# Andreas-Edling/raytracer-rs

Hardware: AMD Instinct MI355X
Metric: Mrays/s (whole node) + ms/frame, 1920x1080x64spp thai2.dae (higher is better)
Workload: dtype f32

## Files before the change

### raytracer-rs_amd/csrc/lightmap.cpp

```cpp
#include "lightmap.hpp"
#include <algorithm>
#include <cmath>
#include <cstring>
#include <limits>

namespace mi355rt {
namespace {

struct V3 { double x, y, z; };
inline V3 sub(V3 a, V3 b) { return { a.x - b.x, a.y - b.y, a.z - b.z }; }
inline V3 add(V3 a, V3 b) { return { a.x + b.x, a.y + b.y, a.z + b.z }; }
inline V3 mul(V3 a, double s) { return { a.x * s, a.y * s, a.z * s }; }
inline double dot(V3 a, V3 b) { return a.x * b.x + a.y * b.y + a.z * b.z; }
inline V3 cross(V3 a, V3 b) { return { a.y * b.z - a.z * b.y, a.z * b.x - a.x * b.z, a.x * b.y - a.y * b.x }; }
inline double len(V3 a) { return std::sqrt(dot(a, a)); }
inline double comp(V3 a, int k) { return k == 0 ? a.x : k == 1 ? a.y : a.z; }

double origin_triangle_distance(V3 a, V3 b, V3 c)
{
    const V3 ab = sub(b, a), ac = sub(c, a), ap = mul(a, -1.0);
    const double d1 = dot(ab, ap), d2 = dot(ac, ap);
    if (d1 <= 0.0 && d2 <= 0.0) return len(a);
    const V3 bp = mul(b, -1.0);
    const double d3 = dot(ab, bp), d4 = dot(ac, bp);
    if (d3 >= 0.0 && d4 <= d3) return len(b);
    const double vc = d1 * d4 - d3 * d2;
    if (vc <= 0.0 && d1 >= 0.0 && d3 <= 0.0) return len(add(a, mul(ab, d1 / (d1 - d3))));
    const V3 cp = mul(c, -1.0);
    const double d5 = dot(ab, cp), d6 = dot(ac, cp);
    if (d6 >= 0.0 && d5 <= d6) return len(c);
    const double vb = d5 * d2 - d1 * d6;
    if (vb <= 0.0 && d2 >= 0.0 && d6 <= 0.0) return len(add(a, mul(ac, d2 / (d2 - d6))));
    const double va = d3 * d6 - d5 * d4;
    if (va <= 0.0 && (d4 - d3) >= 0.0 && (d5 - d6) >= 0.0) return len(add(b, mul(sub(c, b), (d4 - d3) / ((d4 - d3) + (d5 - d6)))));
    const double den = va + vb + vc;
    if (!(std::fabs(den) > 0.0)) return -1.0;
    const double v = vb / den, w = vc / den;
    return len(add(a, add(mul(ab, v), mul(ac, w))));
}

template <class F> int clip(const V3* in, int n, V3* out, F f)
{
    int m = 0;
    for (int i = 0; i < n; ++i) {
        const V3 A = in[i], B = in[(i + 1) % n];
        const double fa = f(A), fb = f(B);
        if (fa >= 0.0) out[m++] = A;
        if ((fa >= 0.0) != (fb >= 0.0)) { const double t = fa / (fa - fb); out[m++] = add(A, mul(sub(B, A), t)); }
    }
    return m;
}

inline float round_down(double v)
{
    float f = (float)v;
    if ((double)f > v) f = std::nextafterf(f, 0.0f);
    return f;
}

}

static const int kAxisA[3] = { 1, 0, 0 }, kAxisB[3] = { 2, 2, 1 };

void build_light_map(const float* tri_verts, uint32_t ntri, const float light[3], double pad, uint32_t res, LightMap& out)
{
    const uint32_t R = res;
    out.res = R;
    out.dist2.assign((size_t)6 * R * R, std::numeric_limits<float>::infinity());
    out.nearest = std::numeric_limits<double>::infinity();
    const V3 L = { light[0], light[1], light[2] };
    const double rho = std::sqrt(2.0) / (double)R * 1.001;
    const double cos_rho = std::cos(rho), sin_rho = std::sin(rho);
    for (uint32_t t = 0; t < ntri; ++t) {
        const float* v = tri_verts + 9 * (size_t)t;
        const V3 P[3] = { sub({ v[0], v[1], v[2] }, L), sub({ v[3], v[4], v[5] }, L), sub({ v[6], v[7], v[8] }, L) };
        double dmin = origin_triangle_distance(P[0], P[1], P[2]);
        {
            const double size = std::max(len(sub(P[1], P[0])), std::max(len(sub(P[2], P[0])), len(sub(P[2], P[1]))));
            const double near_vertex = std::min(len(P[0]), std::min(len(P[1]), len(P[2])));
            const double lower = std::max(near_vertex - size, 0.0);
            if (!(dmin >= 0.0) || !std::isfinite(dmin)) dmin = lower;
            dmin = std::min(std::max(dmin, lower), near_vertex);
            if (!(dmin == dmin)) dmin = 0.0;
        }
        out.nearest = std::min(out.nearest, dmin);
        const V3 n = cross(sub(P[1], P[0]), sub(P[2], P[0]));
        const double nn = len(n);
        const bool has_plane = nn > 0.0 && std::isfinite(nn);
        double h = 0.0; V3 nh = { 0, 0, 0 };
        if (has_plane) { const double c = dot(n, P[0]) / nn; h = std::fabs(c); nh = mul(n, (c < 0.0 ? -1.0 : 1.0) / nn); }
        for (int face = 0; face < 6; ++face) {
            const int m = face >> 1, a = kAxisA[m], b = kAxisB[m];
            const double sg = (face & 1) ? -1.0 : 1.0;
            V3 poly[2][16]; int np = 3;
            poly[0][0] = P[0]; poly[0][1] = P[1]; poly[0][2] = P[2];
            const double eps = 1e-12 * (1.0 + len(P[0])), dl = 1e-6;
            int cur = 0;
            np = clip(poly[cur], np, poly[cur ^ 1], [&](V3 q) { return sg * comp(q, m) - eps; }); cur ^= 1; if (np == 0) continue;
            np = clip(poly[cur], np, poly[cur ^ 1], [&](V3 q) { return sg * comp(q, m) * (1.0 + dl) - comp(q, a); }); cur ^= 1; if (np == 0) continue;
            np = clip(poly[cur], np, poly[cur ^ 1], [&](V3 q) { return sg * comp(q, m) * (1.0 + dl) + comp(q, a); }); cur ^= 1; if (np == 0) continue;
            np = clip(poly[cur], np, poly[cur ^ 1], [&](V3 q) { return sg * comp(q, m) * (1.0 + dl) - comp(q, b); }); cur ^= 1; if (np == 0) continue;
            np = clip(poly[cur], np, poly[cur ^ 1], [&](V3 q) { return sg * comp(q, m) * (1.0 + dl) + comp(q, b); }); cur ^= 1; if (np == 0) continue;
            double u0 = 1e300, u1 = -1e300, v0 = 1e300, v1 = -1e300, mmin = 1e300;
            for (int k = 0; k < np; ++k) {
                const double mm = sg * comp(poly[cur][k], m);
                if (!(mm > 0.0)) { mmin = 0.0; continue; }
                mmin = std::min(mmin, mm);
                const double uu = comp(poly[cur][k], a) / mm, vv = comp(poly[cur][k], b) / mm;
                u0 = std::min(u0, uu); u1 = std::max(u1, uu); v0 = std::min(v0, vv); v1 = std::max(v1, vv);
            }
            long i0 = 0, i1 = (long)R - 1, j0 = 0, j1 = (long)R - 1;
            if (mmin > 0.0 && u0 <= u1) {
                const double mu = 2.5 * pad / mmin + 1e-7;
                i0 = (long)std::floor((std::max(u0 - mu, -1.0) * 0.5 + 0.5) * R - 0.01); i1 = (long)std::floor((std::min(u1 + mu, 1.0) * 0.5 + 0.5) * R + 0.01);
                j0 = (long)std::floor((std::max(v0 - mu, -1.0) * 0.5 + 0.5) * R - 0.01); j1 = (long)std::floor((std::min(v1 + mu, 1.0) * 0.5 + 0.5) * R + 0.01);
                i0 = std::max(i0, 0L); j0 = std::max(j0, 0L); i1 = std::min(i1, (long)R - 1); j1 = std::min(j1, (long)R - 1);
            }
            float* fm = out.dist2.data() + (size_t)face * R * R;
            for (long i = i0; i <= i1; ++i) {
                const double uc = ((double)i + 0.5) / R * 2.0 - 1.0;
                for (long j = j0; j <= j1; ++j) {
                    double lb = dmin;
                    if (has_plane) {
                        const double vc = ((double)j + 0.5) / R * 2.0 - 1.0;
                        double w[3]; w[m] = sg; w[a] = uc; w[b] = vc;
                        const double wl = std::sqrt(w[0] * w[0] + w[1] * w[1] + w[2] * w[2]);
                        const double cos_c = (w[0] * nh.x + w[1] * nh.y + w[2] * nh.z) / wl;
                        if (cos_c > -0.999999) {
                            const double sin_c = std::sqrt(std::max(0.0, 1.0 - cos_c * cos_c));
                            const double cos_lo = cos_c >= cos_rho ? 1.0 : cos_c * cos_rho + sin_c * sin_rho;
                            if (cos_lo > 1e-4) lb = std::max(lb, h / cos_lo);
                            else lb = std::max(lb, h * 1e4);
                        }
                    }
                    const double d = std::max(lb - pad, 0.0);
                    const float val = round_down(d * d * (1.0 - 1e-6));
                    float& dst = fm[(size_t)i * R + (size_t)j];
                    if (val < dst) dst = val;
                }
            }
        }
    }
}

double point_triangle_distance_lower(const double p[3], const float* v)
{
    const V3 L = { p[0], p[1], p[2] };
    const V3 P[3] = { sub({ v[0], v[1], v[2] }, L), sub({ v[3], v[4], v[5] }, L), sub({ v[6], v[7], v[8] }, L) };
    double dmin = origin_triangle_distance(P[0], P[1], P[2]);
    const double size = std::max(len(sub(P[1], P[0])), std::max(len(sub(P[2], P[0])), len(sub(P[2], P[1]))));
    const double near_vertex = std::min(len(P[0]), std::min(len(P[1]), len(P[2])));
    const double lower = std::max(near_vertex - size, 0.0);
    if (!(dmin >= 0.0) || !std::isfinite(dmin)) dmin = lower;
    dmin = std::min(std::max(dmin, lower), near_vertex);
    return dmin == dmin ? dmin : 0.0;
}

uint64_t light_map_work(const float* tri_verts, uint32_t ntri, const float light[3], uint32_t res)
{
    const V3 L = { light[0], light[1], light[2] };
    double total = 0.0;
    for (uint32_t t = 0; t < ntri; ++t) {
        const float* v = tri_verts + 9 * (size_t)t;
        const V3 P[3] = { sub({ v[0], v[1], v[2] }, L), sub({ v[3], v[4], v[5] }, L), sub({ v[6], v[7], v[8] }, L) };
        const V3 c = mul(add(P[0], add(P[1], P[2])), 1.0 / 3.0);
        const double r = std::max(len(sub(P[0], c)), std::max(len(sub(P[1], c)), len(sub(P[2], c)))), d = len(c);
        double frac = 1.0;
        if (d > r * 1.0001) { const double s = r / d; frac = std::min(1.0, s * s * 0.5 + 4.0 / ((double)res * res)); }
        total += frac * 6.0 * (double)res * res;
    }
    return (uint64_t)std::min(total, 1e18);
}

}
```

### raytracer-rs_amd/csrc/reflmask.hpp

```cpp
#pragma once
#include <cstdint>
#include <vector>

namespace mi355rt {

constexpr double kReflMinCos = 0.05;
constexpr double kReflPadAngle = 1e-3;
constexpr float kReflBary = 0.02f;
constexpr double kReflHeightUlps = 16.0;
constexpr uint32_t kReflBins = 8;
constexpr uint32_t kReflGuardWords = 4;

struct ReflMask {
    uint32_t bins = 0;
    uint32_t stride = 0;
    std::vector<uint32_t> words;
    double build_ms = 0.0;
    uint64_t work = 0;
    uint64_t exact_tests = 0;
    uint64_t clear_bits = 0;
};

inline uint32_t refl_mask_stride(uint32_t bins) { return 6u * bins * bins / 32u + kReflGuardWords; }

bool build_reflect_mask(const float* tri_verts, uint32_t ntri, double pad, uint32_t bins, uint64_t work_budget, ReflMask& out,
                        double min_cos = kReflMinCos, double pad_angle = kReflPadAngle);

}
```

### raytracer-rs_amd/csrc/renderer.cpp

```cpp
#include "renderer.hpp"
#include "display.hpp"
#include "lightmap.hpp"
#include "reflmask.hpp"
#include <algorithm>
#include <array>
#include <chrono>
#include <cmath>
#include <cstdio>
#include <cstdlib>
#include <cstring>
#include "kernels.hpp"
#include "lens.hpp"
#include "octree.hpp"

namespace mi355rt {

namespace {
void pcg4d(uint32_t v[4])
{
    for (int i = 0; i < 4; ++i) v[i] = v[i] * 1664525u + 1013904223u;
    v[0] += v[1] * v[3]; v[1] += v[2] * v[0]; v[2] += v[0] * v[1]; v[3] += v[1] * v[2];
    for (int i = 0; i < 4; ++i) v[i] ^= v[i] >> 16;
    v[0] += v[1] * v[3]; v[1] += v[2] * v[0]; v[2] += v[0] * v[1]; v[3] += v[1] * v[2];
}
float u01(uint32_t bits) { return (float)(bits >> 9) * (1.0f / 8388608.0f); }
}

bool Renderer::fail(hipError_t e, const char* what)
{
    last_error = std::string(what) + ": " + hipGetErrorString(e);
    return false;
}
#define HIP_TRY(expr) do { hipError_t e__ = (expr); if (e__ != hipSuccess) return fail(e__, #expr); } while (0)

bool Renderer::bind()
{
    HIP_TRY(hipSetDevice(cfg.device));
    return true;
}

template <class T> bool Renderer::upload(DeviceBuffer<T>& buf, const void* src, size_t bytes)
{
    HIP_TRY(buf.alloc(bytes ? bytes : 16, &hbm_bytes_));
    if (bytes && src) HIP_TRY(hipMemcpy(buf.get(), src, bytes, hipMemcpyHostToDevice));
    else if (bytes) HIP_TRY(hipMemset(buf.get(), 0, bytes));
    return true;
}

template <class T> bool Renderer::upload(T*& dptr, const void* src, size_t bytes)
{
    scene_bufs_.emplace_back();
    if (!upload(scene_bufs_.back(), src, bytes)) return false;
    dptr = static_cast<T*>(scene_bufs_.back().get());
    return true;
}

std::unique_ptr<Renderer> Renderer::create(const SceneData& scene, const mi355rt_config& cfg, std::string& err, int& code)
{
    std::unique_ptr<Renderer> r(new Renderer());
    r->cfg = cfg;
    if (!r->init(scene, err, code)) return nullptr;
    return r;
}

void Renderer::build_sample_table(std::vector<float>& table4)
{
    table.resize((size_t)kNumSamples * 3);
    table4.assign((size_t)kNumSamples * 4, 0.0f);
    for (uint32_t i = 0; i < kNumSamples; ++i) {
        for (uint32_t attempt = 0;; ++attempt) {
            uint32_t h[4] = { i, attempt, 0xFFFFFFFFu, (uint32_t)cfg.seed };
            pcg4d(h);
            Vec3 d(u01(h[0]) * 2.0f + -1.0f, u01(h[1]) * 2.0f + -1.0f, u01(h[2]) * 2.0f + -1.0f);
            if (dot(d, d) < 1.0f) {
                Vec3 nrm = d.normalized();
                table[3 * (size_t)i] = nrm.x; table[3 * (size_t)i + 1] = nrm.y; table[3 * (size_t)i + 2] = nrm.z;
                table4[4 * (size_t)i] = nrm.x; table4[4 * (size_t)i + 1] = nrm.y; table4[4 * (size_t)i + 2] = nrm.z;
                break;
            }
        }
    }
}

bool Renderer::set_seed(uint64_t seed)
{
    if (!bind()) return false;
    if (!settle_speculation()) return false;
    cfg.seed = seed;
    std::vector<float> table4;
    build_sample_table(table4);
    for (Slice& o : slices_) if (o.stream) HIP_TRY(hipStreamSynchronize(o.stream));
    HIP_TRY(hipMemcpy(const_cast<void*>(dscene_.table), table4.data(), table4.size() * sizeof(float), hipMemcpyHostToDevice));
    return true;
}

bool Renderer::set_flags(uint32_t flags)
{
    constexpr uint32_t kCreateMask = MI355RT_FLAG_OCTREE_SEMANTICS | MI355RT_FLAG_TRUE_CLOSEST_HIT | MI355RT_FLAG_GROUP_SHARES_DEVICE | MI355RT_FLAG_DEVICE_LBVH | MI355RT_FLAG_DIRECT_FILM;
    if ((flags ^ cfg.flags) & kCreateMask) { last_error = "the intersector flags (OCTREE_SEMANTICS, TRUE_CLOSEST_HIT), GROUP_SHARES_DEVICE, DEVICE_LBVH and DIRECT_FILM are create-time flags: they cannot be changed with mi355rt_set_flags"; return false; }
    if (flags != cfg.flags && !settle_speculation()) return false;
    cfg.flags = flags;
    return true;
}

bool Renderer::init(const SceneData& scene, std::string& err, int& code)
{
    code = MI355RT_E_INVALID;
    if (cfg.recursions == 0 && cfg.spread == 0) { cfg.recursions = 2; cfg.spread = 1; }
    if (cfg.spread == 0) cfg.spread = 1;
    if (cfg.triangles_per_leaf == 0) cfg.triangles_per_leaf = MI355RT_DEFAULT_TRIANGLES_PER_LEAF;
    if (cfg.width == 0 || cfg.height == 0) { err = "width and height must be non-zero"; return false; }
    if ((uint64_t)cfg.width * cfg.height > 0x7FFFFFFFull / 4) { err = "image too large"; return false; }
    if (cfg.recursions > kMaxRecursions) { err = "recursions > 3 not supported"; return false; }
    if (scene.cameras.empty()) { err = "scene has no camera"; return false; }
    if (scene.tri_geom.size() * 9 != scene.tri_verts.size()) { err = "tri_verts / tri_geom size mismatch"; return false; }
    for (uint32_t g : scene.tri_geom) if (g >= scene.materials.size()) { err = "tri_geom entry out of range"; return false; }
    for (auto& m : scene.materials) if (m.kind == 1 && m.tex_id >= scene.textures.size()) { err = "material texture id out of range"; return false; }
    if (scene.tri_geom.size() >= (1u << 26)) { err = "too many triangles"; return false; }
    {
        uint64_t count = 1, first = 0;
        for (uint32_t l = 0; l <= cfg.recursions; ++l) {
            level_first[l] = (uint32_t)first; first += count; count *= (uint64_t)cfg.spread * (cfg.recursions - l);
            if (first > 0xFFFF) { err = "radiance tree too large (spread * recursions)"; return false; }
        }
        for (uint32_t l = cfg.recursions + 1; l <= kMaxLevels; ++l) level_first[l] = (uint32_t)first;
        nodes_per_sample = (uint32_t)first;
    }
    if (cfg.stripe_world <= 1) { cfg.stripe_world = 1; cfg.stripe_rank = 0; }
    if (cfg.stripe_rows == 0) cfg.stripe_rows = MI355RT_DEFAULT_STRIPE_ROWS;
    if (cfg.stripe_rank >= cfg.stripe_world) { err = "stripe_rank >= stripe_world"; return false; }

    code = MI355RT_E_NO_DEVICE;
    int ndev = 0;
    hipError_t e = hipGetDeviceCount(&ndev);
    if (e != hipSuccess || ndev <= 0) { err = std::string("no HIP device available (") + hipGetErrorString(e) + "); this library has no CPU fallback"; return false; }
    if (cfg.device < 0 || cfg.device >= ndev) { err = "HIP device ordinal out of range"; return false; }
    auto bail = [&]() { err = last_error; return false; };
    if (!bind()) return bail();
    hipDeviceProp_t prop;
    if (hipGetDeviceProperties(&prop, cfg.device) != hipSuccess) { err = "hipGetDeviceProperties failed"; return false; }
    num_cus_ = prop.multiProcessorCount > 0 ? prop.multiProcessorCount : 256;
    if (hipStreamCreateWithFlags(&stream_, hipStreamNonBlocking) != hipSuccess) { err = "hipStreamCreate failed"; return false; }
    if (hipEventCreate(&ev_begin_) != hipSuccess || hipEventCreate(&ev_end_) != hipSuccess) { err = "hipEventCreate failed"; return false; }

    ntri = scene.ntri();
    nlights_ = (uint32_t)scene.lights.size();
    camera = Camera::from_orientation_matrix(cfg.width, cfg.height, Matrix::from_array(scene.cameras[0].orientation), scene.cameras[0].fov_deg);

    const auto t_bvh = std::chrono::steady_clock::now();
    bool on_device = false;
    if (cfg.flags & MI355RT_FLAG_DEVICE_LBVH) {
        std::string why; double ms[2];
        on_device = build_bvh_device(scene.tri_verts.data(), scene.tri_geom.data(), ntri, bvh, why, ms);
        if (on_device) { lbvh_device_ms_ = ms[0]; }
        else last_error = "device LBVH not used (" + why + "): host SAH build instead";
    }
    if (!on_device) build_bvh(scene.tri_verts.data(), scene.tri_geom.data(), ntri, bvh);
    bvh_on_device_ = on_device;
    wide_ = false;
    if (kernels_walk_wide_nodes()) {
        build_wide(bvh);
        if (!bvh.nodes4.empty()) wide_ = true;
        else if (bvh.root >= 0) { err = "this build's kernels walk the 4-wide tree, which does not serve this scene"; code = MI355RT_E_INVALID; return false; }
    }
    build_ms_[0] = std::chrono::duration<double, std::milli>(std::chrono::steady_clock::now() - t_bvh).count();
    collect_cull_boxes();
    if (bvh.max_depth > kBvhMaxDepth) { err = "internal: BVH deeper than the traversal stack"; code = MI355RT_E_INVALID; return false; }
    std::vector<float> normals((size_t)std::max(ntri, 1u) * 4, 0.0f);
    for (uint32_t t = 0; t < ntri; ++t) {
        const float* v = &scene.tri_verts[9 * (size_t)t];
        Vec3 v0(v[0], v[1], v[2]), v1(v[3], v[4], v[5]), v2(v[6], v[7], v[8]);
        Vec3 n = cross(v1 - v0, v2 - v0).normalized();
        normals[4 * (size_t)t] = n.x; normals[4 * (size_t)t + 1] = n.y; normals[4 * (size_t)t + 2] = n.z;
        uint32_t g = scene.tri_geom[t];
        std::memcpy(&normals[4 * (size_t)t + 3], &g, 4);
    }
    std::vector<float> table4;
    build_sample_table(table4);
    void* d_nodes = nullptr; void* d_tris = nullptr; void* d_normals = nullptr; void* d_table = nullptr;
    DMaterial* d_mats = nullptr; DLight* d_lights = nullptr; DTexture* d_tex = nullptr; float* d_texels = nullptr;
    if (wide_ ? !upload(d_nodes, bvh.nodes4.data(), bvh.nodes4.size() * sizeof(BvhNode4)) : !upload(d_nodes, bvh.nodes.data(), bvh.nodes.size() * sizeof(BvhNode))) return bail();
    if (!upload(d_tris, bvh.tris.data(), bvh.tris.size() * sizeof(BvhTri))) return bail();
    if (!upload(d_normals, normals.data(), normals.size() * sizeof(float))) return bail();
    if (!upload(d_table, table4.data(), table4.size() * sizeof(float))) return bail();
    std::vector<DMaterial> mats(std::max<size_t>(scene.materials.size(), 1));
    for (size_t i = 0; i < scene.materials.size(); ++i) {
        const MaterialData& m = scene.materials[i];
        mats[i] = DMaterial{ m.rgb[0], m.rgb[1], m.rgb[2], m.kind == 1 ? (0x80000000u | m.tex_id) : 0u };
    }
    if (!upload(d_mats, mats.data(), mats.size() * sizeof(DMaterial))) return bail();
    std::vector<DLight> lights(std::max<size_t>(scene.lights.size(), 1));
    for (size_t i = 0; i < scene.lights.size(); ++i) {
        const LightData& l = scene.lights[i];
        lights[i] = DLight{ l.pos[0], l.pos[1], l.pos[2], l.color[0], l.color[1], l.color[2], 0.0f, 0.0f };
    }
    float* d_light_maps = nullptr; uint32_t light_map_res = 0;
    if (!scene.lights.empty() && scene.lights.size() <= 8 && ntri > 0 && !getenv("MI355RT_NO_LIGHT_MAP")) {
        const auto t_lm = std::chrono::steady_clock::now();
        double diag2 = 0.0;
        { float mn[3] = { 3e38f, 3e38f, 3e38f }, mx[3] = { -3e38f, -3e38f, -3e38f };
          for (size_t i = 0; i < scene.tri_verts.size(); ++i) { const int a = (int)(i % 3); mn[a] = std::min(mn[a], scene.tri_verts[i]); mx[a] = std::max(mx[a], scene.tri_verts[i]); }
          for (int a = 0; a < 3; ++a) diag2 += ((double)mx[a] - mn[a]) * ((double)mx[a] - mn[a]); }
        const double pad = 2e-4 * std::sqrt(diag2) + 1e-7;
        uint32_t res = 512;
        while (res > 16 && (size_t)6 * res * res * 4 * scene.lights.size() > ((size_t)64 << 20)) res /= 2;
        const uint64_t work_cap = 4ull << 20;
        for (const LightData& l : scene.lights) while (res > 16 && light_map_work(scene.tri_verts.data(), ntri, l.pos, res) > work_cap) res /= 2;
        std::vector<float> all; all.reserve((size_t)6 * res * res * scene.lights.size());
        bool finite = true;
        for (size_t i = 0; i < scene.lights.size() && finite; ++i) {
            const LightData& l = scene.lights[i];
            if (!std::isfinite(l.pos[0]) || !std::isfinite(l.pos[1]) || !std::isfinite(l.pos[2])) { finite = false; break; }
            LightMap lm; build_light_map(scene.tri_verts.data(), ntri, l.pos, pad, res, lm);
            all.insert(all.end(), lm.dist2.begin(), lm.dist2.end());
            const double tail = std::max(lm.nearest - pad, 0.0);
            lights[i].tail2 = std::isfinite(tail) ? (float)std::min(tail * tail * (1.0 - 1e-6), 3.0e38) : 3.0e38f;
            if ((double)lights[i].tail2 > tail * tail) lights[i].tail2 = std::nextafterf(lights[i].tail2, 0.0f);
        }
        if (finite) {
            if (!upload(d_light_maps, all.data(), all.size() * sizeof(float))) return bail();
            light_map_res = res;
        }
        light_map_ms_ = std::chrono::duration<double, std::milli>(std::chrono::steady_clock::now() - t_lm).count();
        if (getenv("MI355RT_DEBUG_CULL")) fprintf(stderr, "[mi355rt] light maps: %zu lights, %u texels per face edge, %.1f ms\n", scene.lights.size(), light_map_res, light_map_ms_);
    }
    if (!upload(d_lights, lights.data(), lights.size() * sizeof(DLight))) return bail();
    uint32_t* d_refl_mask = nullptr; uint32_t refl_bins = 0, refl_stride = 0;
    if (ntri > 0 && cfg.recursions > 0 && !getenv("MI355RT_NO_REFLECT_MASK")) {
        double diag2 = 0.0;
        { float mn[3] = { 3e38f, 3e38f, 3e38f }, mx[3] = { -3e38f, -3e38f, -3e38f };
          for (size_t i = 0; i < scene.tri_verts.size(); ++i) { const int a = (int)(i % 3); mn[a] = std::min(mn[a], scene.tri_verts[i]); mx[a] = std::max(mx[a], scene.tri_verts[i]); }
          for (int a = 0; a < 3; ++a) diag2 += ((double)mx[a] - mn[a]) * ((double)mx[a] - mn[a]); }
        uint64_t budget = 4000000000ull;
        if (const char* e = getenv("MI355RT_REFLECT_MASK_WORK")) budget = std::strtoull(e, nullptr, 10);
        ReflMask rm;
        if (std::isfinite(diag2) && build_reflect_mask(scene.tri_verts.data(), ntri, 2e-4 * std::sqrt(diag2) + 1e-7, kReflBins, budget, rm)) {
            if (!upload(d_refl_mask, rm.words.data(), rm.words.size() * sizeof(uint32_t))) return bail();
            refl_bins = rm.bins; refl_stride = rm.stride;
            reflect_mask_info_[2] = (double)rm.clear_bits / ((double)ntri * 6.0 * rm.bins * rm.bins);
            reflect_mask_info_[3] = (double)(rm.words.size() * sizeof(uint32_t));
        }
        reflect_mask_info_[0] = (double)refl_bins; reflect_mask_info_[1] = rm.build_ms;
        if (getenv("MI355RT_DEBUG_CULL")) fprintf(stderr, "[mi355rt] reflection masks: %u bins per face edge, %.1f ms, %llu work units, %.3f of the bits clear\n", refl_bins, rm.build_ms, (unsigned long long)rm.work, reflect_mask_info_[2]);
    }
    std::vector<DTexture> tex(std::max<size_t>(scene.textures.size(), 1));
    std::vector<float> texels;
    for (size_t i = 0; i < scene.textures.size(); ++i) {
        const TextureData& t = scene.textures[i];
        if (t.rgb.size() != (size_t)t.width * t.height * 3 || t.rgb.empty()) { err = "texture size mismatch"; code = MI355RT_E_INVALID; return false; }
        tex[i] = DTexture{ t.width, t.height, texels.size() / 3 };
        texels.insert(texels.end(), t.rgb.begin(), t.rgb.end());
    }
    if (!upload(d_tex, tex.data(), tex.size() * sizeof(DTexture))) return bail();
    if (!upload(d_texels, texels.data(), texels.size() * sizeof(float))) return bail();
    dscene_.nodes = d_nodes; dscene_.tris = d_tris; dscene_.normals = d_normals; dscene_.materials = d_mats;
    dscene_.lights = d_lights; dscene_.textures = d_tex; dscene_.texels = d_texels; dscene_.table = d_table;
    dscene_.root = bvh.root; dscene_.nlights = nlights_; dscene_.ntri = ntri;
    dscene_.light_maps = d_light_maps; dscene_.light_map_res = light_map_res;
    dscene_.refl_mask = d_refl_mask; dscene_.refl_bins = refl_bins; dscene_.refl_stride = refl_stride;
    dscene_.oct_nodes = nullptr; dscene_.oct_leaf_tris = nullptr; dscene_.prim_tris = nullptr; dscene_.oct_info = nullptr; dscene_.tri_home = nullptr; dscene_.oct_single_leaf = 0u;
    std::memset(dscene_.oct_root, 0, sizeof dscene_.oct_root);
    mode_ = (cfg.flags & MI355RT_FLAG_OCTREE_SEMANTICS) ? kModeOctreeWalk : (cfg.flags & MI355RT_FLAG_TRUE_CLOSEST_HIT) ? kModeTrueClosest : kModeConfirm;
    if (mode_ != kModeTrueClosest) {
        Octree oct;
        const auto t_oct = std::chrono::steady_clock::now();
        build_octree(scene.tri_verts.data(), ntri, cfg.triangles_per_leaf, oct);
        build_ms_[1] = std::chrono::duration<double, std::milli>(std::chrono::steady_clock::now() - t_oct).count();
        oct_stats_[0] = (uint32_t)oct.nodes.size(); oct_stats_[1] = oct.inner; oct_stats_[2] = oct.leaves;
        oct_stats_[3] = oct.empty_leaves; oct_stats_[4] = oct.max_depth; oct_stats_[5] = (uint32_t)oct.leaf_tris.size();
        std::vector<BvhTri> prim_tris(std::max(ntri, 1u));
        std::memset(prim_tris.data(), 0, prim_tris.size() * sizeof(BvhTri));
        for (uint32_t t = 0; t < ntri; ++t) {
            const float* v = &scene.tri_verts[9 * (size_t)t];
            for (int a = 0; a < 3; ++a) { prim_tris[t].v0[a] = v[a]; prim_tris[t].e1[a] = v[3 + a] - v[a]; prim_tris[t].e2[a] = v[6 + a] - v[a]; }
            prim_tris[t].prim = t; prim_tris[t].geom = scene.tri_geom[t];
        }
        void* d_oct = nullptr; uint32_t* d_leaf = nullptr; void* d_ptris = nullptr;
        if (!upload(d_oct, oct.nodes.data(), oct.nodes.size() * sizeof(OctNodeFlat))) return bail();
        if (!upload(d_leaf, oct.leaf_tris.data(), oct.leaf_tris.size() * 4)) return bail();
        if (!upload(d_ptris, prim_tris.data(), prim_tris.size() * sizeof(BvhTri))) return bail();
        dscene_.oct_nodes = d_oct; dscene_.oct_leaf_tris = d_leaf; dscene_.prim_tris = d_ptris;
        std::vector<int2> info(oct.nodes.size());
        std::vector<uint32_t> home(std::max(ntri, 1u), 0xFFFFFFFEu);
        for (size_t i = 0; i < oct.nodes.size(); ++i) {
            const OctNodeFlat& f = oct.nodes[i];
            if (f.first_child >= 0) { info[i].x = f.first_child; info[i].y = 0; continue; }
            info[i].x = ~(int32_t)f.tri_first; info[i].y = (int32_t)f.tri_count;
            for (uint32_t k = 0; k < f.tri_count; ++k) {
                uint32_t& h = home[oct.leaf_tris[f.tri_first + k]];
                h = h == 0xFFFFFFFEu ? (uint32_t)i : 0xFFFFFFFFu;
            }
        }
        int2* d_info = nullptr; uint32_t* d_home = nullptr;
        if (!upload(d_info, info.data(), info.size() * sizeof(int2))) return bail();
        if (!upload(d_home, home.data(), home.size() * 4)) return bail();
        dscene_.oct_info = d_info; dscene_.tri_home = d_home;
        dscene_.oct_single_leaf = (mode_ == kModeConfirm && oct.nodes.size() == 1) ? 1u : 0u;
        for (int a = 0; a < 3; ++a) { dscene_.oct_root[a] = oct.nodes[0].cmin[a]; dscene_.oct_root[3 + a] = oct.nodes[0].cmax[a]; }
    }

    const size_t npix = (size_t)cfg.width * cfg.height;
    if (!upload(d_film_sum_, nullptr, npix * 12) || !upload(d_film_sumsq_, nullptr, npix * 12) || !upload(d_film_n_, nullptr, npix * 4)) return bail();
    if ((cfg.flags & MI355RT_FLAG_DIRECT_FILM) && !upload(d_film_direct_, nullptr, npix * 12)) return bail();
    if (!upload(d_ldr_, nullptr, npix * 4)) return bail();
    ldr_dirty_.assign(cfg.height, (uint8_t)1);
    if (hipEventCreateWithFlags(&ev_tonemap_, hipEventDisableTiming) != hipSuccess || hipEventCreateWithFlags(&ev_gather_, hipEventDisableTiming) != hipSuccess) { err = "hipEventCreate failed"; return false; }
    if (hipEventCreateWithFlags(&ev_call_done_, hipEventDisableTiming) != hipSuccess || hipEventCreateWithFlags(&ev_spec_done_, hipEventDisableTiming) != hipSuccess
        || hipStreamCreateWithFlags(&read_stream_, hipStreamNonBlocking) != hipSuccess) { err = "hipEventCreate / hipStreamCreate failed"; return false; }
    std::vector<uint32_t> all(cfg.height);
    for (uint32_t r = 0; r < cfg.height; ++r) {
        all[r] = r;
        if ((r / cfg.stripe_rows) % cfg.stripe_world == cfg.stripe_rank) owned_rows.push_back(r);
    }
    if (!upload(d_all_rows_, all.data(), all.size() * 4)) return bail();
    if (!upload(d_owned_rows_, owned_rows.data(), owned_rows.size() * 4)) return bail();
    if (!upload(d_tmp_rows_, nullptr, 64 * 4)) return bail();
    if (!upload(d_counters_, nullptr, sizeof(DCounters) * kShards)) return bail();
    if (h_counters_.alloc(sizeof(DCounters) * kShards) != hipSuccess) { err = "pinned host allocation failed"; return false; }
    std::memset(h_counters_.get(), 0, sizeof(DCounters) * kShards);
    slices_[0].stream = stream_;
    for (uint32_t i = 0; i < kMaxSlices; ++i) {
        if (i && hipStreamCreateWithFlags(&slices_[i].stream, hipStreamNonBlocking) != hipSuccess) { err = "hipStreamCreate failed"; return false; }
        if (hipEventCreateWithFlags(&slices_[i].done, hipEventDisableTiming) != hipSuccess) { err = "hipEventCreate failed"; return false; }
        if (!upload(slices_[i].d_ctrl, nullptr, kMaxRounds * kCtrlWordsPerRound * 4)) return bail();
        if (!upload(slices_[i].d_rows, nullptr, (size_t)cfg.height * 4)) return bail();
    }
    if (const char* e = getenv("MI355RT_SLICES")) { int v = atoi(e); if (v >= 1 && v <= (int)kMaxSlices) slices = (uint32_t)v; }
    if (!upload(d_debug_color_, nullptr, 16)) return bail();

    records_per_sample_ = 1;
    for (uint32_t l = 0; l <= cfg.recursions; ++l) {
        uint32_t nl = level_first[l + 1] - level_first[l];
        uint32_t nn = l < cfg.recursions ? level_first[l + 2] - level_first[l + 1] : 0;
        records_per_sample_ = std::max(records_per_sample_, nl * std::max(nlights_, 1u) + nn);
    }
    max_level_nodes_ = 1;
    for (uint32_t l = 0; l <= cfg.recursions; ++l) max_level_nodes_ = std::max(max_level_nodes_, level_first[l + 1] - level_first[l]);
    code = MI355RT_OK;
    return true;
}

Renderer::~Renderer()
{
    if (hipSetDevice(cfg.device) != hipSuccess) return;
    if (stream_) (void)hipStreamSynchronize(stream_);
    if (read_stream_) (void)hipStreamSynchronize(read_stream_);
    for (uint32_t i = 0; i < kMaxSlices; ++i) {
        if (i && slices_[i].stream) { (void)hipStreamSynchronize(slices_[i].stream); (void)hipStreamDestroy(slices_[i].stream); }
        if (slices_[i].done) (void)hipEventDestroy(slices_[i].done);
    }
    comm_destroy();
    if (ev_tonemap_) (void)hipEventDestroy(ev_tonemap_);
    if (read_stream_) (void)hipStreamDestroy(read_stream_);
    if (ev_call_done_) (void)hipEventDestroy(ev_call_done_);
    if (ev_spec_done_) (void)hipEventDestroy(ev_spec_done_);
    if (ev_gather_) (void)hipEventDestroy(ev_gather_);
    for (hipEvent_t e : ev_pool_) (void)hipEventDestroy(e);
    if (ev_begin_) (void)hipEventDestroy(ev_begin_);
    if (ev_end_) (void)hipEventDestroy(ev_end_);
    if (stream_) (void)hipStreamDestroy(stream_);
}

void Renderer::collect_cull_boxes()
{
    cull_boxes_.clear();
    if (ntri == 0) return;
    auto half_to_float = [](uint32_t h) {
        _Float16 v; uint16_t b = (uint16_t)h; std::memcpy(&v, &b, 2); return (float)v;
    };
    struct Item { std::array<float, 6> box; int32_t node; };
    std::vector<Item> items;
    Item root; root.node = bvh.root;
    for (int a = 0; a < 3; ++a) { root.box[a] = bvh.scene_min[a]; root.box[3 + a] = bvh.scene_max[a]; }
    items.push_back(root);
    for (;;) {
        int best = -1; float best_size = -1.0f;
        for (size_t i = 0; i < items.size(); ++i) {
            if (items[i].node < 0) continue;
            const auto& b = items[i].box;
            const float size = (b[3] - b[0]) * (b[4] - b[1]) + (b[4] - b[1]) * (b[5] - b[2]) + (b[5] - b[2]) * (b[3] - b[0]);
            if (size > best_size) { best_size = size; best = (int)i; }
        }
        if (best < 0 || items.size() + 1 > kCullRects) break;
        const BvhNode& n = bvh.nodes[items[best].node];
        Item c0, c1;
        for (int a = 0; a < 3; ++a) {
            c0.box[a] = half_to_float(n.h0[a] & 0xFFFFu); c0.box[3 + a] = half_to_float(n.h0[a] >> 16);
            c1.box[a] = half_to_float(n.h1[a] & 0xFFFFu); c1.box[3 + a] = half_to_float(n.h1[a] >> 16);
        }
        c0.node = n.child0; c1.node = n.child1;
        items[best] = c0;
        items.push_back(c1);
    }
    for (const Item& it : items) {
        bool finite = true;
        for (float v : it.box) if (!std::isfinite(v)) finite = false;
        if (!finite) { cull_boxes_.clear(); return; }
        cull_boxes_.push_back(it.box);
    }
}

bool Renderer::project_triangles(const DCamera& c, const double inv[3][3], double pad, double zmin)
{
    std::vector<float> key(c.rot, c.rot + 16);
    key.insert(key.end(), c.origin, c.origin + 3);
    if (key == rects_key_ && tri_rects_.size() == bvh.tris.size()) return rects_ok_;
    rects_key_ = key; rects_ok_ = false;
    tri_rects_.resize(bvh.tris.size());
    const double kx = std::fabs(inv[0][0]) + std::fabs(inv[1][0]) + std::fabs(inv[2][0]), ky = std::fabs(inv[0][1]) + std::fabs(inv[1][1]) + std::fabs(inv[2][1]);
    const double kz = std::fabs(inv[0][2]) + std::fabs(inv[1][2]) + std::fabs(inv[2][2]);
    for (size_t i = 0; i < bvh.tris.size(); ++i) {
        const BvhTri& t = bvh.tris[i];
        double x0 = 1e300, x1 = -1e300, y0 = 1e300, y1 = -1e300;
        for (int v = 0; v < 3; ++v) {
            double w[3];
            for (int a = 0; a < 3; ++a) w[a] = (double)t.v0[a] + (v == 1 ? (double)t.e1[a] : v == 2 ? (double)t.e2[a] : 0.0) - c.origin[a];
            const double vx = w[0] * inv[0][0] + w[1] * inv[1][0] + w[2] * inv[2][0];
            const double vy = w[0] * inv[0][1] + w[1] * inv[1][1] + w[2] * inv[2][1];
            const double vz = w[0] * inv[0][2] + w[1] * inv[1][2] + w[2] * inv[2][2] - pad * kz;
            if (!(vz > zmin)) return false;
            const double dx = vx / (vz + pad * kz), dy = -vy / (vz + pad * kz);
            const double mx = pad * (kx + std::fabs(dx) * kz) / vz * 1.0001 + 4e-16 * (1.0 + std::fabs(dx)), my = pad * (ky + std::fabs(dy) * kz) / vz * 1.0001 + 4e-16 * (1.0 + std::fabs(dy));
            x0 = std::min(x0, dx - mx); x1 = std::max(x1, dx + mx); y0 = std::min(y0, dy - my); y1 = std::max(y1, dy + my);
        }
        tri_rects_[i] = TriRect{ x0, x1, y0, y1 };
    }
    rects_ok_ = true;
    return true;
}

bool Renderer::refresh_cull_mask(DCamera& c, const double inv[3][3], double pad, double zmin, bool build)
{
    c.cull_mask = nullptr; c.mask_x0 = c.mask_y0 = 0.0f; c.mask_inv_cx = c.mask_inv_cy = 0.0f;
    if (c.cull_valid == 0 || bvh.tris.empty() || bvh.tris.size() > (2u << 20) || getenv("MI355RT_NO_CULL_MASK")) return true;
    std::vector<float> key(c.rot, c.rot + 16);
    key.insert(key.end(), c.origin, c.origin + 3); key.push_back(c.max_x); key.push_back(c.max_y);
    if (key == mask_key_) {
        if (mask_valid_) { c.cull_mask = d_cull_mask_.get(); c.mask_x0 = mask_dom_[0]; c.mask_y0 = mask_dom_[1]; c.mask_inv_cx = mask_dom_[2]; c.mask_inv_cy = mask_dom_[3]; }
        return true;
    }
    if (!build) return true;
    mask_key_ = key; mask_valid_ = false;
    double X0 = 1e300, X1 = -1e300, Y0 = 1e300, Y1 = -1e300;
    for (uint32_t k = 0; k < c.cull_valid; ++k) { X0 = std::min(X0, (double)c.cull_rect[k][0]); X1 = std::max(X1, (double)c.cull_rect[k][1]); Y0 = std::min(Y0, (double)c.cull_rect[k][2]); Y1 = std::max(Y1, (double)c.cull_rect[k][3]); }
    if (!(X1 > X0) || !(Y1 > Y0)) return true;
    const double icx = kCullGrid / (X1 - X0), icy = kCullGrid / (Y1 - Y0);
    constexpr uint32_t wpr = kCullGrid / 32u;
    std::vector<uint32_t> bits((size_t)kCullGrid * wpr, 0u);
    if (!project_triangles(c, inv, pad, zmin)) return true;
    for (const TriRect& tr : tri_rects_) {
        const double x0 = tr.x0, x1 = tr.x1, y0 = tr.y0, y1 = tr.y1;
        const double mx = 1e-4 * (x1 - x0) + 1e-6, my = 1e-4 * (y1 - y0) + 1e-6;
        const long i0 = std::max(0L, (long)std::floor((x0 - mx - X0) * icx - 0.01)), i1 = std::min((long)kCullGrid - 1, (long)std::floor((x1 + mx - X0) * icx + 0.01));
        const long j0 = std::max(0L, (long)std::floor((y0 - my - Y0) * icy - 0.01)), j1 = std::min((long)kCullGrid - 1, (long)std::floor((y1 + my - Y0) * icy + 0.01));
        for (long j = j0; j <= j1; ++j) for (long i = i0; i <= i1; ++i) bits[(size_t)j * wpr + (size_t)(i >> 5)] |= 1u << (i & 31);
    }
    if (!bind()) return false;
    if (!d_cull_mask_ && d_cull_mask_.alloc(bits.size() * 4, &hbm_bytes_) != hipSuccess) return true;
    (void)hipStreamSynchronize(stream_);
    for (Slice& sl : slices_) if (sl.stream) (void)hipStreamSynchronize(sl.stream);
    if (hipMemcpy(d_cull_mask_.get(), bits.data(), bits.size() * 4, hipMemcpyHostToDevice) != hipSuccess) return true;
    mask_dom_[0] = (float)X0; mask_dom_[1] = (float)Y0; mask_dom_[2] = (float)icx; mask_dom_[3] = (float)icy;
    mask_valid_ = true;
    c.cull_mask = d_cull_mask_.get(); c.mask_x0 = mask_dom_[0]; c.mask_y0 = mask_dom_[1]; c.mask_inv_cx = mask_dom_[2]; c.mask_inv_cy = mask_dom_[3];
    if (getenv("MI355RT_DEBUG_CULL")) { size_t n = 0; for (uint32_t w : bits) n += (size_t)__builtin_popcount(w); fprintf(stderr, "[mi355rt] cull mask: %zu of %u cells set, domain x [%g, %g] y [%g, %g]\n", n, kCullGrid * kCullGrid, X0, X1, Y0, Y1); }
    return true;
}

bool Renderer::refresh_tile_bins(DCamera& c, const double inv[3][3], double pad, double zmin, const DPass& ps, const std::vector<uint32_t>& rows)
{
#define BINS_OUT(k) do { if (getenv("MI355RT_DEBUG_CULL")) fprintf(stderr, "[mi355rt] tile bins: not built (exit %d)\n", k); return true; } while (0)
    c.tile_ofs = nullptr; c.tile_entries = nullptr; c.tile_cols = c.tile_rg = c.tile_nblocks = 0;
    if (c.cull_valid == 0 || bvh.tris.empty() || bvh.tris.size() > (2u << 20) || getenv("MI355RT_NO_RASTER")) BINS_OUT(1);
    const uint32_t W = cfg.width, H = cfg.height, rg = ps.row_group, G = ps.sample_group;
    if (ps.use_explicit || G == 0 || 64u % G || (64u / G) % rg || ps.chunk % 64u) BINS_OUT(2);
    const uint32_t cols = 64u / G / rg;
    if (W % cols || rows.size() % rg || rows.empty() || ps.npix != rows.size() * (size_t)W) BINS_OUT(3);
    for (size_t i = 0; i < rows.size(); i += rg) {
        if (rows[i] % rg) BINS_OUT(4);
        for (uint32_t k = 1; k < rg; ++k) if (rows[i + k] != rows[i] + k) BINS_OUT(5);
    }
    const bool fix_row = (ps.flags & 1u) != 0;
    std::vector<float> key(c.rot, c.rot + 16);
    key.insert(key.end(), c.origin, c.origin + 3); key.push_back(c.max_x); key.push_back(c.max_y);
    key.push_back((float)cols); key.push_back((float)rg); key.push_back(fix_row ? 1.0f : 0.0f);
    const uint32_t nblocks = W / cols, ngroups = (H + rg - 1) / rg;
    auto publish = [&]() { c.tile_ofs = d_tile_ofs_.get(); c.tile_entries = d_tile_entries_.get(); c.tile_cols = cols; c.tile_rg = rg; c.tile_nblocks = nblocks; };
    if (key == bins_key_) { if (bins_valid_) publish(); return true; }
    bins_key_ = key; bins_valid_ = false;
    const auto t_begin = std::chrono::steady_clock::now();
    const double mx = c.max_x, my = c.max_y;
    const uint64_t vmax = fix_row ? (uint64_t)H - 1 : ((uint64_t)W * H - 1) / H;
    struct Ref { uint32_t tile; float dmin; uint32_t tri; };
    std::vector<Ref> refs;
    refs.reserve(bvh.tris.size() * 6);
    const double org[3] = { c.origin[0], c.origin[1], c.origin[2] };
    if (!project_triangles(c, inv, pad, zmin)) BINS_OUT(7);
    for (size_t k = 0; k < bvh.tris.size(); ++k) {
        const BvhTri& t = bvh.tris[k];
        float v9[9];
        for (int a = 0; a < 3; ++a) { v9[a] = t.v0[a]; v9[3 + a] = t.v0[a] + t.e1[a]; v9[6 + a] = t.v0[a] + t.e2[a]; }
        const double x0 = tri_rects_[k].x0, x1 = tri_rects_[k].x1, y0 = tri_rects_[k].y0, y1 = tri_rects_[k].y1;
        const double ex = 1e-4 * (x1 - x0) + 1e-6, ey = 1e-4 * (y1 - y0) + 1e-6;
        const double fx0 = (x0 - ex + mx) / (2.0 * mx) * W - 0.01, fx1 = (x1 + ex + mx) / (2.0 * mx) * W + 0.01;
        const double fy0 = (y0 - ey + my) / (2.0 * my) * H - 0.01, fy1 = (y1 + ey + my) / (2.0 * my) * H + 0.01;
        if (fx1 < 0.0 || fx0 >= (double)W || fy1 < 0.0 || fy0 > (double)vmax + 1.0) continue;
        const uint64_t c0 = (uint64_t)std::max(0.0, std::floor(fx0)), c1 = (uint64_t)std::min((double)W - 1.0, std::floor(fx1));
        const uint64_t v0 = (uint64_t)std::max(0.0, std::floor(fy0)), v1 = (uint64_t)std::min((double)vmax, std::floor(fy1));
        if (c1 < c0 || v1 < v0) continue;
        uint64_t r0, r1;
        if (fix_row) { r0 = v0; r1 = std::min<uint64_t>(v1, H - 1); }
        else {
            const uint64_t lo = v0 * H, hi = (v1 + 1) * H - 1;
            r0 = lo > c1 ? (lo - c1 + W - 1) / W : 0; r1 = hi >= c0 ? (hi - c0) / W : 0;
            if (hi < c0) continue;
            r1 = std::min<uint64_t>(r1, H - 1);
        }
        if (r1 < r0) continue;
        const double org_d = point_triangle_distance_lower(org, v9);
        const float dmin = (float)std::max((org_d - pad) * (1.0 - 1e-6), 0.0);
        const float dmin_lo = (double)dmin > std::max((org_d - pad) * (1.0 - 1e-6), 0.0) ? std::nextafterf(dmin, 0.0f) : dmin;
        for (uint64_t g = r0 / rg; g <= r1 / rg && g < ngroups; ++g) {
            const uint64_t ra = g * rg, rb = std::min<uint64_t>(ra + rg - 1, H - 1);
            for (uint64_t b = c0 / cols; b <= c1 / cols; ++b) {
                const uint64_t xa = b * cols, xb = xa + cols - 1;
                const uint64_t ta = fix_row ? ra : (ra * W + xa) / H, tb = fix_row ? rb : (rb * W + xb) / H;
                if (tb < v0 || ta > v1) continue;
                refs.push_back(Ref{ (uint32_t)(g * nblocks + b), dmin_lo, (uint32_t)k });
            }
        }
    }
    const size_t ntiles = (size_t)nblocks * ngroups;
    std::vector<uint2> ofs(ntiles, make_uint2(0u, 0u));
    for (const Ref& r : refs) ++ofs[r.tile].y;
    size_t live = 0; uint32_t run = 0;
    for (uint2& o : ofs) { o.x = run; run += o.y; live += o.y != 0; o.y = 0; }
    if (refs.size() > ((size_t)64 << 20) || (live && refs.size() > 24 * live)) BINS_OUT(8);
    std::vector<uint2> entries(std::max<size_t>(refs.size(), 1));
    for (const Ref& r : refs) { uint2& o = ofs[r.tile]; uint32_t bits; std::memcpy(&bits, &r.dmin, 4); entries[o.x + o.y++] = make_uint2(r.tri, bits); }
// ... 1124 lines not shown
```

Baseline: 20560.

## Multithread light-map build, skip dominated texels, and double reflection-mask bins

The host light-map construction now runs in two multithreaded phases. The first clips triangles against each cube face and records texel rectangles per thread. The second splits each face into row bands and fills texels band by band, skipping a texel early when its stored value already beats the triangle's distance floor. Separately, the default reflection-mask resolution rises from 8 to 16 bins, and environment overrides are added for light-map resolution and mask bins. Finer masks should cull more reflection rays on the GPU, at the cost of more host build time and a larger mask to upload and read.

```diff
diff --git a/raytracer-rs_amd/csrc/lightmap.cpp b/raytracer-rs_amd/csrc/lightmap.cpp
--- a/raytracer-rs_amd/csrc/lightmap.cpp
+++ b/raytracer-rs_amd/csrc/lightmap.cpp
@@ -1,8 +1,12 @@
 #include "lightmap.hpp"
 #include <algorithm>
+#include <atomic>
 #include <cmath>
+#include <cstdlib>
 #include <cstring>
 #include <limits>
+#include <thread>
+#include <vector>
 
 namespace mi355rt {
 namespace {
@@ -62,6 +66,28 @@
 
 static const int kAxisA[3] = { 1, 0, 0 }, kAxisB[3] = { 2, 2, 1 };
 
+namespace {
+
+struct TriBound { double dmin, h; V3 nh; bool has_plane; };
+struct FaceRect { uint32_t tri; uint16_t i0, i1, j0, j1; };
+
+uint32_t light_map_threads(uint64_t units)
+{
+    uint32_t n = std::min(16u, std::thread::hardware_concurrency());
+    if (const char* e = std::getenv("MI355RT_LIGHT_MAP_THREADS")) { const int v = std::atoi(e); if (v >= 1 && v <= 16) n = (uint32_t)v; }
+    return (uint32_t)std::max<uint64_t>(1u, std::min<uint64_t>(n, units));
+}
+
+template <class F> void run_on(uint32_t nthreads, F worker)
+{
+    std::vector<std::thread> pool;
+    for (uint32_t i = 1; i < nthreads; ++i) pool.emplace_back(worker, i);
+    worker(0u);
+    for (std::thread& th : pool) th.join();
+}
+
+}
+
 void build_light_map(const float* tri_verts, uint32_t ntri, const float light[3], double pad, uint32_t res, LightMap& out)
 {
     const uint32_t R = res;
@@ -71,7 +97,12 @@
     const V3 L = { light[0], light[1], light[2] };
     const double rho = std::sqrt(2.0) / (double)R * 1.001;
     const double cos_rho = std::cos(rho), sin_rho = std::sin(rho);
-    for (uint32_t t = 0; t < ntri; ++t) {
+    std::vector<TriBound> bounds(ntri);
+    const uint32_t nt1 = light_map_threads((ntri + 4095u) / 4096u);
+    std::vector<std::vector<FaceRect>> rects((size_t)nt1 * 6);
+    std::vector<double> nearest(nt1, std::numeric_limits<double>::infinity());
+    std::atomic<uint32_t> next{ 0 };
+    auto triangle = [&](uint32_t t, uint32_t me) {
         const float* v = tri_verts + 9 * (size_t)t;
         const V3 P[3] = { sub({ v[0], v[1], v[2] }, L), sub({ v[3], v[4], v[5] }, L), sub({ v[6], v[7], v[8] }, L) };
         double dmin = origin_triangle_distance(P[0], P[1], P[2]);
@@ -83,12 +114,13 @@
             dmin = std::min(std::max(dmin, lower), near_vertex);
             if (!(dmin == dmin)) dmin = 0.0;
         }
-        out.nearest = std::min(out.nearest, dmin);
+        nearest[me] = std::min(nearest[me], dmin);
         const V3 n = cross(sub(P[1], P[0]), sub(P[2], P[0]));
         const double nn = len(n);
         const bool has_plane = nn > 0.0 && std::isfinite(nn);
         double h = 0.0; V3 nh = { 0, 0, 0 };
         if (has_plane) { const double c = dot(n, P[0]) / nn; h = std::fabs(c); nh = mul(n, (c < 0.0 ? -1.0 : 1.0) / nn); }
+        bounds[t] = TriBound{ dmin, h, nh, has_plane };
         for (int face = 0; face < 6; ++face) {
             const int m = face >> 1, a = kAxisA[m], b = kAxisB[m];
             const double sg = (face & 1) ? -1.0 : 1.0;
@@ -116,31 +148,68 @@
                 j0 = (long)std::floor((std::max(v0 - mu, -1.0) * 0.5 + 0.5) * R - 0.01); j1 = (long)std::floor((std::min(v1 + mu, 1.0) * 0.5 + 0.5) * R + 0.01);
                 i0 = std::max(i0, 0L); j0 = std::max(j0, 0L); i1 = std::min(i1, (long)R - 1); j1 = std::min(j1, (long)R - 1);
             }
+            if (i0 <= i1 && j0 <= j1) rects[(size_t)me * 6 + face].push_back(FaceRect{ t, (uint16_t)i0, (uint16_t)i1, (uint16_t)j0, (uint16_t)j1 });
+        }
+    };
+    run_on(nt1, [&](uint32_t me) {
+        for (;;) {
+            const uint32_t first = next.fetch_add(1024u);
+            if (first >= ntri) break;
+            for (uint32_t t = first; t < std::min(first + 1024u, ntri); ++t) triangle(t, me);
+        }
+    });
+    for (double d : nearest) out.nearest = std::min(out.nearest, d);
+    const uint32_t band_rows = std::max(1u, R / 128u), nbands = (R + band_rows - 1u) / band_rows;
+    std::vector<std::vector<const FaceRect*>> bands((size_t)6 * nbands);
+    for (uint32_t th = 0; th < nt1; ++th) for (int face = 0; face < 6; ++face)
+        for (const FaceRect& r : rects[(size_t)th * 6 + face])
+            for (uint32_t bd = r.i0 / band_rows; bd <= r.i1 / band_rows; ++bd) bands[(size_t)face * nbands + bd].push_back(&r);
+    uint64_t updates = 0;
+    for (const auto& rs : rects) for (const FaceRect& r : rs) updates += (uint64_t)(r.i1 - r.i0 + 1u) * (r.j1 - r.j0 + 1u);
+    std::atomic<uint32_t> next_band{ 0 };
+    auto texels = [&](uint32_t) {
+        for (;;) {
+            const uint32_t unit = next_band.fetch_add(1u);
+            if (unit >= 6u * nbands) break;
+            const int face = (int)(unit / nbands);
+            const long row0 = (long)(unit % nbands) * band_rows, row1 = std::min(row0 + (long)band_rows, (long)R) - 1;
+            const int m = face >> 1, a = kAxisA[m], b = kAxisB[m];
+            const double sg = (face & 1) ? -1.0 : 1.0;
             float* fm = out.dist2.data() + (size_t)face * R * R;
-            for (long i = i0; i <= i1; ++i) {
-                const double uc = ((double)i + 0.5) / R * 2.0 - 1.0;
-                for (long j = j0; j <= j1; ++j) {
-                    double lb = dmin;
-                    if (has_plane) {
-                        const double vc = ((double)j + 0.5) / R * 2.0 - 1.0;
-                        double w[3]; w[m] = sg; w[a] = uc; w[b] = vc;
-                        const double wl = std::sqrt(w[0] * w[0] + w[1] * w[1] + w[2] * w[2]);
-                        const double cos_c = (w[0] * nh.x + w[1] * nh.y + w[2] * nh.z) / wl;
-                        if (cos_c > -0.999999) {
-                            const double sin_c = std::sqrt(std::max(0.0, 1.0 - cos_c * cos_c));
-                            const double cos_lo = cos_c >= cos_rho ? 1.0 : cos_c * cos_rho + sin_c * sin_rho;
-                            if (cos_lo > 1e-4) lb = std::max(lb, h / cos_lo);
-                            else lb = std::max(lb, h * 1e4);
+            for (const FaceRect* r : bands[unit]) {
+                const TriBound& tb = bounds[r->tri];
+                const double dmin = tb.dmin, h = tb.h; const V3 nh = tb.nh;
+                const bool has_plane = tb.has_plane && h > 0.0;
+                const double d0 = std::max(dmin - pad, 0.0);
+                const float floor_val = round_down(d0 * d0 * (1.0 - 1e-6));
+                for (long i = std::max((long)r->i0, row0); i <= std::min((long)r->i1, row1); ++i) {
+                    const double uc = ((double)i + 0.5) / R * 2.0 - 1.0;
+                    for (long j = r->j0; j <= (long)r->j1; ++j) {
+                        float& dst = fm[(size_t)i * R + (size_t)j];
+                        if (dst <= floor_val) continue;
+                        if (!has_plane) { dst = floor_val; continue; }
+                        double lb = dmin;
+                        {
+                            const double vc = ((double)j + 0.5) / R * 2.0 - 1.0;
+                            double w[3]; w[m] = sg; w[a] = uc; w[b] = vc;
+                            const double wl = std::sqrt(w[0] * w[0] + w[1] * w[1] + w[2] * w[2]);
+                            const double cos_c = (w[0] * nh.x + w[1] * nh.y + w[2] * nh.z) / wl;
+                            if (cos_c > -0.999999) {
+                                const double sin_c = std::sqrt(std::max(0.0, 1.0 - cos_c * cos_c));
+                                const double cos_lo = cos_c >= cos_rho ? 1.0 : cos_c * cos_rho + sin_c * sin_rho;
+                                if (cos_lo > 1e-4) lb = std::max(lb, h / cos_lo);
+                                else lb = std::max(lb, h * 1e4);
+                            }
                         }
+                        const double d = std::max(lb - pad, 0.0);
+                        const float val = round_down(d * d * (1.0 - 1e-6));
+                        if (val < dst) dst = val;
                     }
-                    const double d = std::max(lb - pad, 0.0);
-                    const float val = round_down(d * d * (1.0 - 1e-6));
-                    float& dst = fm[(size_t)i * R + (size_t)j];
-                    if (val < dst) dst = val;
                 }
             }
         }
-    }
+    };
+    run_on(light_map_threads(std::max<uint64_t>(1u, updates >> 16)), texels);
 }
 
 double point_triangle_distance_lower(const double p[3], const float* v)
diff --git a/raytracer-rs_amd/csrc/reflmask.hpp b/raytracer-rs_amd/csrc/reflmask.hpp
--- a/raytracer-rs_amd/csrc/reflmask.hpp
+++ b/raytracer-rs_amd/csrc/reflmask.hpp
@@ -8,7 +8,7 @@
 constexpr double kReflPadAngle = 1e-3;
 constexpr float kReflBary = 0.02f;
 constexpr double kReflHeightUlps = 16.0;
-constexpr uint32_t kReflBins = 8;
+constexpr uint32_t kReflBins = 16;
 constexpr uint32_t kReflGuardWords = 4;
 
 struct ReflMask {
diff --git a/raytracer-rs_amd/csrc/renderer.cpp b/raytracer-rs_amd/csrc/renderer.cpp
--- a/raytracer-rs_amd/csrc/renderer.cpp
+++ b/raytracer-rs_amd/csrc/renderer.cpp
@@ -202,10 +202,12 @@
           for (size_t i = 0; i < scene.tri_verts.size(); ++i) { const int a = (int)(i % 3); mn[a] = std::min(mn[a], scene.tri_verts[i]); mx[a] = std::max(mx[a], scene.tri_verts[i]); }
           for (int a = 0; a < 3; ++a) diag2 += ((double)mx[a] - mn[a]) * ((double)mx[a] - mn[a]); }
         const double pad = 2e-4 * std::sqrt(diag2) + 1e-7;
-        uint32_t res = 512;
+        uint32_t res = 512, forced = 0;
+        if (const char* e = getenv("MI355RT_LIGHT_MAP_RES")) { const long v = atol(e); if (v >= 16 && v <= 2048 && (v & (v - 1)) == 0) forced = (uint32_t)v; }
         while (res > 16 && (size_t)6 * res * res * 4 * scene.lights.size() > ((size_t)64 << 20)) res /= 2;
         const uint64_t work_cap = 4ull << 20;
-        for (const LightData& l : scene.lights) while (res > 16 && light_map_work(scene.tri_verts.data(), ntri, l.pos, res) > work_cap) res /= 2;
+        for (const LightData& l : scene.lights) while (!forced && res > 16 && light_map_work(scene.tri_verts.data(), ntri, l.pos, res) > work_cap) res /= 2;
+        if (forced) res = forced;
         std::vector<float> all; all.reserve((size_t)6 * res * res * scene.lights.size());
         bool finite = true;
         for (size_t i = 0; i < scene.lights.size() && finite; ++i) {
@@ -234,7 +236,9 @@
         uint64_t budget = 4000000000ull;
         if (const char* e = getenv("MI355RT_REFLECT_MASK_WORK")) budget = std::strtoull(e, nullptr, 10);
         ReflMask rm;
-        if (std::isfinite(diag2) && build_reflect_mask(scene.tri_verts.data(), ntri, 2e-4 * std::sqrt(diag2) + 1e-7, kReflBins, budget, rm)) {
+        uint32_t bins = kReflBins;
+        if (const char* e = getenv("MI355RT_REFLECT_MASK_BINS")) { const int v = atoi(e); if (v == 8 || v == 16) bins = (uint32_t)v; }
+        if (std::isfinite(diag2) && build_reflect_mask(scene.tri_verts.data(), ntri, 2e-4 * std::sqrt(diag2) + 1e-7, bins, budget, rm)) {
             if (!upload(d_refl_mask, rm.words.data(), rm.words.size() * sizeof(uint32_t))) return bail();
             refl_bins = rm.bins; refl_stride = rm.stride;
             reflect_mask_info_[2] = (double)rm.clear_bits / ((double)ntri * 6.0 * rm.bins * rm.bins);
```

Result: faster. 20980, median of 6 (+2.1%).
